# emmanuel-ferdman/pinot

Measured on AMD Instinct MI355X. Metric: rows scanned/s (G) + p50 query latency, SSB flattened SF100/SF1000, 1-8 GPU, higher is better.
Workload: dtype u32 dict ids / int64 sums; 1 GPU; SSB SF100 flattened lineorder per GPU, 100 segments x 6000000 rows, queries Q1.1+Q1.2+Q1.3; layout=sorted by LO_ORDERDATE (SURVEY.md §8d C2), rows_per_gpu=600000000, parallelism=one GPU (no collective)

## Files before the change

### pinot_amd/csrc/device.h

```cpp
#pragma once
#include <stdint.h>

#if defined(__HIPCC__)
#define PHIP_HD __host__ __device__
#else
#define PHIP_HD
#endif

namespace phip {

constexpr int kMaxQueryColumns = 16;
constexpr int kMaxAggs = 8;
constexpr int kRecKeys = 4;
constexpr int kRecFields = kRecKeys + 2 * kMaxAggs;
enum { REC_BITS = 0, REC_U16 = 1, REC_U32 = 2 };
struct RecSrc {
  const void *p;
  int32_t kind, bits, off, pad;
};
struct RecSrcs {
  RecSrc f[kRecFields];
};
constexpr int kMaxPrograms = 8;
constexpr int kDenseMin = 640;
constexpr int kDoneSlot = 63;
constexpr int kMaxFilterStack = 6;
constexpr int kMaxGroupBy = 8;
constexpr int kWave = 64;
constexpr int kTileGroups = 32;
constexpr int kTileDocs = kTileGroups * 64;
constexpr int kMaxStage = 8;
constexpr int kStagePad = 16;
constexpr int kMaxHllRegs = 1 << 12;

constexpr int kFilterBlock = 256;
constexpr int kFilterWaves = kFilterBlock / kWave;
constexpr int kMaxRing = 8;
constexpr int kFilterStaticLds = 448;
constexpr int kFusedRingTile = 512;
#ifndef PHIP_FUSED_RING_DEFER
#define PHIP_FUSED_RING_DEFER 512
#endif
constexpr int kFusedRingDefer = PHIP_FUSED_RING_DEFER;
constexpr int kAggBlock = 512;
constexpr int kAggWaves = kAggBlock / kWave;
#ifndef PHIP_KBATCH
#define PHIP_KBATCH 4
#endif
constexpr int kRingAgg = PHIP_KBATCH <= 4 ? 1024 : 2048;
constexpr int kRingGroup = 128;
constexpr int kRingGroupBatch = PHIP_KBATCH <= 4 ? 512 : 1024;
constexpr int kFusedRingGB = 256;
constexpr int kFusedBatchGB = 2;
constexpr int ring_entries(int mode, bool batched = false) {
  return mode == 0 ? kRingAgg : (batched ? kRingGroupBatch : kRingGroup);
}
constexpr int kMaxAggStage = 4;
constexpr int kAggStageBudget = 4096;
constexpr int kAggLdsDict = 1024;

enum AccKind : int32_t {
  ACC_COUNT = 0,
  ACC_SUM_I64 = 1,
  ACC_SUM_F64 = 2,
  ACC_MIN_F64 = 3,
  ACC_MAX_F64 = 4,
  ACC_HLL = 5,
  ACC_DISTINCT = 6,
};

enum DevOp : int32_t { DOP_LEAF = 0, DOP_AND = 1, DOP_OR = 2, DOP_NOT = 3 };
enum SkipKind : int32_t { SKIP_NONE = 0, SKIP_IF_NONE = 1, SKIP_IF_ALL = 2 };

enum GroupMode : int32_t {
  GB_NONE = 0,
  GB_LDS = 1,
  GB_GLOBAL = 2,
  GB_HASH = 3,
  GB_XCD = 4,
};
constexpr int kXcdCopies = 8;
constexpr int kFusedGroupBy = -1;
constexpr int kFusedGroupByXcd = -2;
constexpr int kFusedGroupByLds = -3;
constexpr uint64_t kHashEmpty = ~0ull;

struct DevCol {
  const uint32_t *words;
  const void *dict;
  const void *raw;
  const int32_t *remap;
  const uint32_t *hll;
  int32_t bits;
  int32_t card;
  int32_t type;
  int32_t has_dict;
  int32_t lds_off;
  int32_t hll_rows;
  const uint64_t *str_off;
  const uint32_t *planes;
  int64_t gb_base;
  const uint32_t *hll_doc;
  const uint16_t *hll_doc16;
  const uint64_t *gb_nulls;
  int64_t gb_null_id;
  const int32_t *gb_ids;
  const uint32_t *vpack;
  int64_t vbase;
  int32_t vbits;
  int32_t vpad;
};
constexpr int kBitSliceMaxBits = 12;

constexpr int kExprMaxOps = 32;
constexpr int kExprMaxStack = 8;
constexpr int kExprMaxCols = 8;
constexpr int kMaxDerivedPerSegment = 16;
enum ExprOp : int32_t { EXOP_COLUMN = 0, EXOP_CONST = 1, EXOP_ADD = 2, EXOP_SUB = 3, EXOP_MUL = 4, EXOP_DIV = 5 };
struct DevExprOp {
  int32_t op;
  int32_t col;
  int64_t lval;
  double dval;
};
struct DevExpr {
  int32_t num_ops;
  int32_t num_docs;
  DevExprOp ops[kExprMaxOps];
  DevCol cols[kExprMaxCols];
};

struct MvScanTask {
  const uint32_t *words;
  const uint32_t *offsets;
  const uint32_t *set;
  uint64_t *out;
  int32_t tile_words;
  int32_t num_docs;
  int32_t num_tiles;
  int32_t tile_begin;
  int32_t bits;
  int32_t lo, hi;
  int32_t invert;
  int32_t set_words;
  int32_t pad;
};
struct MvReduceTask {
  const uint32_t *words;
  const uint32_t *offsets;
  const void *dict;
  void *out;
  int32_t num_docs;
  int32_t bits;
  int32_t type;
  int32_t kind;
  int32_t integral;
  int32_t pad;
};

constexpr int kMaxTupleCols = 8;
constexpr int kMaxTupleWords = 4;
struct TupleCol {
  const uint32_t *words;
  const int32_t *remap;
  const int32_t *ids;
  const void *raw;
  const uint64_t *nulls;
  int64_t base;
  int64_t null_id;
  uint64_t stride;
  int32_t bits;
  int32_t type;
  int32_t word;
  int32_t pad;
};
struct TupleCols {
  TupleCol cols[kMaxTupleCols];
  int32_t k;
  int32_t w;
};

struct StageSrc {
  const uint8_t *base;
  int32_t bytes;
  int32_t lds_off;
};

#ifndef PHIP_MAX_CONJ
#define PHIP_MAX_CONJ 6
#endif
constexpr int kMaxConj = PHIP_MAX_CONJ;
constexpr int kConjSparseMax = 6;
constexpr double kConjSparseSel = 1.0 / 16;
struct ConjLeaf {
  int32_t lds_off;
  int32_t bits;
  int32_t kind;
  uint32_t lo;
  uint32_t span;
  int32_t pad;
  uint64_t set_mask;
};

struct DevSeg {
  int32_t num_docs;
  int32_t work_begin;
  int32_t tile0;
  int32_t num_work;
  int32_t node_begin;
  int32_t node_end;
  int32_t num_stage;
  int32_t seg_index;
  int32_t num_dma;
  int32_t conj;
  int32_t conj_p;
  int32_t conj_sparse;
  int32_t conj_path;
  int32_t conj_range;
  int32_t conj_lo;
  int32_t conj_hi;
  int32_t contig;
  int32_t program;
  int32_t fused_defer;
  int32_t conj_bs;
  ConjLeaf conj_leaf[kMaxConj];
  StageSrc stage[kMaxStage];
  DevCol cols[kMaxQueryColumns];
  const uint32_t *rec;
  int32_t rec_words;
  int32_t rec_nf;
  uint8_t rec_off[kRecFields];
  uint8_t rec_bits[kRecFields];
};

struct DevNode {
  int32_t op;
  int32_t leaf_kind;
  int32_t column;
  int32_t lo, hi;
  int32_t exclusive;
  int32_t count;
  int32_t skip_to;
  int32_t skip_kind;
  int32_t lds_off;
  int32_t bits;
  int32_t small_set;
  int32_t aux_stride;
  uint64_t set_mask;
  int32_t bs_nruns;
  uint32_t bs_runs[4];
  const void *aux;
};

constexpr int kFinShards = 16;
constexpr size_t kFinCounterBytes = 64 * (1 + kFinShards);
struct DevFinal {
  const uint64_t *pa;
  const int32_t *ka;
  const uint64_t *pf;
  const int32_t *kf;
  uint64_t *segm;
  uint32_t *hll;
  uint64_t *out;
  uint32_t *counter;
  int32_t nba, na, nbf, nseg, hll_words, pad;
};

struct DevFilter {
  const DevSeg *segs;
// ... 203 lines not shown
```

### pinot_amd/csrc/filter_kernel.h

```cpp
#pragma once
#include <hip/hip_ext.h>

#include "agg_kernel.h"
#include "host_final.h"

namespace phip {

struct Tile {
  int32_t doc0;
  int32_t valid_docs;
  const PHIP_LDS uint8_t *stage;
};

#define PHIP_GROUP_LOOP(PASS_EXPR)                                             \
  const int lane = lane_id();                                                  \
  const int32_t p = lane * B;                                                  \
  const int32_t q = (p - 1) >> 5;                                              \
  const uint32_t s = (uint32_t)(32 * (q + 1) - p);                             \
  const PHIP_LDS uint32_t *wl = w + q;                                         \
  const int32_t gstride = 2 * B;                                               \
  uint32_t r = 0;                                                              \
  _Pragma("unroll 8") for (int g = 0; g < kTileGroups; g++) {                  \
    const uint32_t win = __builtin_amdgcn_alignbit(wl[0], wl[1], s);           \
    wl += gstride;                                                             \
// ... 1071 lines not shown
static_assert(kFusedRingDefer - 64 * lean_batch(1) >= 32 * defer_piece_lanes(kFusedRingDefer - 64 * lean_batch(1)),
              "a piece fits the ring beside a lean batch");

template <int NA, int U = kFusedBatch>
__device__ __forceinline__ void fused_defer(cquery_t &aq, cseg_t &seg, const Tile &t, uint32_t mask,
                                            PHIP_LDS uint32_t *ring, int &head, int &tail, const SmallDict (&sda)[NA],
                                            const SmallDict (&sdb)[NA], uint64_t (&acc)[NA]) {
  constexpr int kDeferPieceLanes = defer_piece_lanes(kFusedRingDefer - 64 * U);
  if (ballot(mask != 0) == 0) return;
  const TileRank r = rank_tile(mask);
  const int head0 = head;
  const int npiece = head - tail + r.total <= kFusedRingDefer ? 1 : 64 / kDeferPieceLanes;
  const int lanes = 64 / npiece;
  for (int p = 0; p < npiece; p++) {
    const int e = __builtin_amdgcn_readlane((int)r.incl, lanes * p + lanes - 1);
    write_ranked<uint32_t, kFusedRingDefer>(r, lanes * p, lanes * (p + 1), -head0, t.doc0, ring);
    head = head0 + e;
    while (head - tail >= 64 * U) {
      fused_flush<NA, U>(aq, seg, ring, tail, 64 * U, sda, sdb, acc);
      tail += 64 * U;
    }
  }
}

constexpr int kGbFlush = 64 * kFusedBatchGB;
static_assert(kFusedRingGB >= 2 * kGbFlush, "a piece of <= kGbFlush docs lands on < kGbFlush pending");

template <int MODE>
__device__ __forceinline__ void fused_flush_gb(cquery_t &aq, cseg_t &seg, const PHIP_LDS uint32_t *ring, int tail, int n,
                                               lds_u64 *tbl, lds_u32 *hll_packed) {
  group_ring_batch<MODE, kFusedBatchGB, kFusedRingGB>(aq, seg, (const lds_u32 *)ring, tail, n, tbl, hll_packed);
}

template <int MODE>
__device__ __forceinline__ void fused_defer_gb(cquery_t &aq, cseg_t &seg, const Tile &t, uint32_t mask,
                                               PHIP_LDS uint32_t *ring, int &head, int &tail, lds_u64 *tbl,
                                               lds_u32 *hll_packed) {
  if (ballot(mask != 0) == 0) return;
  const TileRank r = rank_tile(mask);
  const int head0 = head;
  const int npiece = head - tail + r.total <= kFusedRingGB ? 1 : 16;
  const int lanes = 64 / npiece;
  for (int p = 0; p < npiece; p++) {
    const int e = __builtin_amdgcn_readlane((int)r.incl, lanes * p + lanes - 1);
    write_ranked<uint32_t, kFusedRingGB>(r, lanes * p, lanes * (p + 1), -head0, t.doc0, ring);
    head = head0 + e;
    while (head - tail >= kGbFlush) {
      fused_flush_gb<MODE>(aq, seg, ring, tail, kGbFlush, tbl, hll_packed);
      tail += kGbFlush;
    }
  }
}

#define PHIP_VMW(k) \
  case k: asm volatile("s_waitcnt vmcnt(" #k ")" ::: "memory"); break;
__device__ __forceinline__ void wait_vmcnt_lb(int n) {
  switch (__builtin_amdgcn_readfirstlane(n)) {
    PHIP_VMW(0) PHIP_VMW(1) PHIP_VMW(2) PHIP_VMW(3) PHIP_VMW(4) PHIP_VMW(5) PHIP_VMW(6) PHIP_VMW(7)
    PHIP_VMW(8) PHIP_VMW(9) PHIP_VMW(10) PHIP_VMW(11) PHIP_VMW(12) PHIP_VMW(13) PHIP_VMW(14)
    default: asm volatile("s_waitcnt vmcnt(15)" ::: "memory"); break;
  }
}
#undef PHIP_VMW

template <int kS>
struct StageCursor {
  const uint8_t *ptr[kS];
  int32_t bytes[kS];
  int32_t lds[kS];
  int32_t n;
};

template <int kS>
__device__ __forceinline__ void cursor_load(StageCursor<kS> &c, cseg_t &seg, int32_t tile_in_seg) {
  c.n = seg.num_stage;
#pragma unroll
  for (int i = 0; i < kS; i++) {
    c.ptr[i] = nullptr;
    c.bytes[i] = 0;
    c.lds[i] = 0;
    if (i < c.n) {
      c.bytes[i] = seg.stage[i].bytes;
      c.lds[i] = seg.stage[i].lds_off;
      c.ptr[i] = seg.stage[i].base + (int64_t)tile_in_seg * c.bytes[i];
    }
  }
}

template <int kS>
__device__ __forceinline__ void cursor_issue(StageCursor<kS> &c, uint32_t lbase, int step) {
  const int lane16 = lane_id() * 16;
#pragma unroll
  for (int i = 0; i < kS; i++) {
    if (i < c.n) {
      const uint8_t *g = c.ptr[i] + lane16;
      const uint32_t l = lbase + (uint32_t)c.lds[i];
      const int32_t nb = c.bytes[i];
      for (int off = 0; off < nb; off += 1024) {
        if (off + lane16 < nb) dma16(g + off, l + (uint32_t)off);
      }
      c.ptr[i] += (int64_t)nb * step;
    }
  }
}

template <int NA>
__device__ __forceinline__ void record_store(const DevFilter &q, const uint64_t *part, const uint64_t *apart,
                                             const uint32_t *segrow) {
  const int i = (int)threadIdx.x;
  if (i >= (q.rec_stride >> 3)) return;
  int na = 0;
  if constexpr (NA > 0) na = ((cquery_t *)q.agg)->num_aggs;
  uint64_t v = 0;
  if (i < 2) {
    for (int w = 0; w < kFilterWaves; w++) v += part[w * 2 + i];
  } else if (i < 2 + 2 * na) {
    if constexpr (NA > 0) {
      const int a = (i - 2) >> 1, kind = ((cquery_t *)q.agg)->aggs[a].acc;
      v = apart[a];
      for (int w = 1; w < kFilterWaves; w++) v = acc_combine(kind, v, apart[w * NA + a]);
      v = (i & 1) ? (v >> 48) : v;
    }
  } else {
    const int e = q.rec_first[blockIdx.x] + (i - 2 - 2 * na);
    for (int w = 0; w < kFilterWaves; w++) v += segrow[w * kRecSegSlots + e % kRecSegSlots];
  }
  __hip_atomic_store(q.rec + (((size_t)blockIdx.x * (uint32_t)q.rec_stride) >> 3) + i, rec_word(q.rec_tag, v),
                     __ATOMIC_RELAXED, __HIP_MEMORY_SCOPE_SYSTEM);
}

#ifndef PHIP_FUSED_WAVES
#define PHIP_FUSED_WAVES 5
#endif
template <bool kConjOnly, int NA, bool kBsDefer = false>
__global__ __launch_bounds__(kFilterBlock, kConjOnly ? (NA != 0 ? PHIP_FUSED_WAVES : 6) : 4) void filter_kernel(DevFilter q) {
  static_assert(!kBsDefer || (kConjOnly && NA > 0), "the lean shape is a fused aggregation");
  constexpr int kSConj = kBsDefer ? kMaxConj : (NA > 0 ? kMaxConj + kMaxAggStage : kMaxConj);
  constexpr int kS = kConjOnly ? (kSConj < kMaxStage ? kSConj : kMaxStage) : kMaxStage;
  extern __shared__ __attribute__((aligned(16))) unsigned char smem[];
  const int lane = lane_id();
  const int wave = uniform(threadIdx.x >> 6);
  int begin, end, step;
  if (q.xcd_walk == 1) {
    const int x = blockIdx.x & 7, gx = gridDim.x >> 3;
    begin = (int)((int64_t)q.total_work * x / 8) + (int)(blockIdx.x >> 3) * kFilterWaves + wave;
    end = (int)((int64_t)q.total_work * (x + 1) / 8);
    step = gx * kFilterWaves;
  } else {
    const TileRange r = wave_tile_range(q.xcd_walk, q.total_work, (int)gridDim.x, (int)blockIdx.x, wave, kFilterWaves);
    begin = r.begin;
    end = r.end;
    step = 1;
  }
  const int nbuf = q.nbuf;
  const int stride = q.stage_stride;
  PHIP_LDS uint8_t *ring = (PHIP_LDS uint8_t *)(smem + (size_t)wave * nbuf * stride);
  PHIP_LDS uint8_t *docring_b = (PHIP_LDS uint8_t *)(smem + (size_t)kFilterWaves * nbuf * stride) +
                                (NA != 0 ? (size_t)wave * q.fring_bytes : 0);
  PHIP_LDS uint16_t *docring = (PHIP_LDS uint16_t *)docring_b;
  PHIP_LDS uint32_t *deferring = (PHIP_LDS uint32_t *)docring_b;
  int dhead = 0, dtail = 0;
  const uint32_t ring_lds = __builtin_amdgcn_readfirstlane((uint32_t)(uintptr_t)ring);

  cseg_t *segs = (cseg_t *)q.segs;
  cnode_t *nodes = (cnode_t *)q.nodes;
  uint32_t lane_matched = 0;
  uint64_t scanned = 0;
  uint64_t matched_total = 0;
  const int nd = q.min_dma;
  const int st = kBsDefer ? 0 : (q.mask_out != nullptr ? 1 : 0);
  constexpr int NAX = NA > 0 ? NA : 1;
  constexpr int kB = kBsDefer ? lean_batch(NA) : kFusedBatch;
  constexpr int kGbMode = NA == kFusedGroupByXcd ? GB_XCD : (NA == kFusedGroupByLds ? GB_LDS : GB_GLOBAL);
  lds_u64 *gtbl = nullptr;
  lds_u32 *ghll = nullptr;
  if constexpr (NA == kFusedGroupByLds) {
    cquery_t &aq = *(cquery_t *)q.agg;
    gtbl = (lds_u64 *)(smem + (size_t)kFilterWaves * (nbuf * stride + q.fring_bytes));
    ghll = (lds_u32 *)((PHIP_LDS uint8_t *)gtbl + (size_t)aq.tbl_words * 8);
    const int G = (int)aq.num_groups;
    for (int i = threadIdx.x; i < aq.tbl_words; i += kFilterBlock) {
      const int row = i / G;
      gtbl[i] = (row > 0 && aq.aggs[row - 1].acc == ACC_MIN_F64) ? ~0ull : 0ull;
    }
    for (int i = threadIdx.x; i < aq.hll_words; i += kFilterBlock) ghll[i] = 0;
    __syncthreads();
  }
  __shared__ uint32_t segrow[kFilterWaves][NA >= 0 ? kRecSegSlots : 1];
  if constexpr (NA >= 0) {
    segrow[wave][min(lane, kRecSegSlots - 1)] = 0;
  }
  uint64_t acc[NAX];
  SmallDict sda[NAX], sdb[NAX];
  if constexpr (NA > 0) {
    cquery_t &aq = *(cquery_t *)q.agg;
#pragma unroll
    for (int a = 0; a < NA; a++) {
      acc[a] = a < aq.num_aggs ? acc_init(aq.aggs[a].acc) : 0;
      sda[a] = sdb[a] = SmallDict{0u, 0u, false};
    }
  }

  int pf = begin, pfc = 0, psn = 0, pend = -1, pslot = 0;
  StageCursor<kS> cur;
  cur.n = 0;
#define PHIP_PREFETCH()                                                                         \
  do {                                                                                          \
    if (pf >= pend) {                                                                           \
      while (psn + 1 < q.num_segs && segs[psn].work_begin + segs[psn].num_work <= pf) psn++;    \
      cseg_t &ps = segs[psn];                                                                   \
      pend = ps.work_begin + ps.num_work;                                                       \
      cursor_load<kS>(cur, ps, ps.tile0 + (pf - ps.work_begin));                                \
    }                                                                                           \
    cursor_issue<kS>(cur, ring_lds + (uint32_t)(pslot * stride), step);                         \
    pf += step;                                                                                 \
    pfc++;                                                                                      \
// ... 186 lines not shown
```

### pinot_amd/csrc/runtime.cpp

```cpp
#include <hip/hip_runtime.h>

#include <algorithm>
#include <atomic>
#include <chrono>
#include <condition_variable>
#include <cmath>
#include <cstdarg>
#include <cstdio>
#include <cstring>
#include <functional>
#include <map>
#include <memory>
#include <mutex>
#include <string>
#include <unordered_map>
#include <vector>

#include "../../include/pinot_hip.h"
#include "device.h"
#include "host_final.h"
#include "launch.h"
#include "node.h"

using namespace phip;

static thread_local std::string g_err;

static int32_t fail(int32_t code, const char *fmt, ...) {
  char buf[1024];
  va_list ap;
  va_start(ap, fmt);
  vsnprintf(buf, sizeof(buf), fmt, ap);
  va_end(ap);
  g_err = buf;
  return code;
}

#define HIP_TRY(expr)                                                                         \
  do {                                                                                        \
    hipError_t _e = (expr);                                                                   \
    if (_e != hipSuccess) return fail(PHIP_ERR_HIP, "%s failed: %s", #expr, hipGetErrorString(_e)); \
  } while (0)

static inline int64_t ceil_div(int64_t a, int64_t b) { return (a + b - 1) / b; }
static inline int64_t round_up(int64_t a, int64_t b) { return ceil_div(a, b) * b; }
static inline uint32_t be32(const uint8_t *p) {
  return ((uint32_t)p[0] << 24) | ((uint32_t)p[1] << 16) | ((uint32_t)p[2] << 8) | p[3];
}
static inline uint64_t be64(const uint8_t *p) { return ((uint64_t)be32(p) << 32) | be32(p + 4); }
static inline uint32_t le32(const uint8_t *p) {
  return (uint32_t)p[0] | ((uint32_t)p[1] << 8) | ((uint32_t)p[2] << 16) | ((uint32_t)p[3] << 24);
}
static inline uint16_t le16(const uint8_t *p) { return (uint16_t)(p[0] | (p[1] << 8)); }

static int num_bits_per_value(int32_t max_value) {
  if (max_value <= 1) return 1;
  int b = 0;
  while (max_value > 0) {
    b++;
    max_value >>= 1;
  }
  return b;
}

static int type_width(int32_t t) {
  switch (t) {
    case PHIP_TYPE_INT:
    case PHIP_TYPE_FLOAT: return 4;
    case PHIP_TYPE_LONG:
    case PHIP_TYPE_DOUBLE: return 8;
    default: return 0;
  }
}

static int32_t murmur_hash_long(int64_t data) {
  const uint32_t m = 0x5bd1e995u;
  uint32_t h = 0;
  uint32_t k = (uint32_t)data * m;
  k ^= k >> 24;
  h ^= k * m;
  k = (uint32_t)((uint64_t)data >> 32) * m;
  k ^= k >> 24;
  h *= m;
  h ^= k * m;
  h ^= h >> 13;
  h *= m;
  h ^= h >> 15;
  return (int32_t)h;
}
static int32_t murmur_hash_bytes(const uint8_t *d, int32_t len, int32_t seed) {
  const uint32_t m = 0x5bd1e995u;
  uint32_t h = (uint32_t)seed ^ (uint32_t)len;
  int32_t n4 = len >> 2;
  for (int32_t i = 0; i < n4; i++) {
    uint32_t k = le32(d + 4 * i);
    k *= m;
    k ^= k >> 24;
    k *= m;
    h *= m;
    h ^= k;
  }
// ... 3636 lines not shown
  int64_t mv_total_tiles = 0, mv_entries = 0;
  for (size_t i = 0; i < inv_leaves.size(); i++) {
    const InvLeaf &L = inv_leaves[i];
    const ColumnStore &cs = segs[L.seg]->cols[L.col];
    uint64_t *words = (uint64_t *)inv_words + inv_word_off[i];
    const int32_t tile_words = 32 * entry_leaves[L.entry];
    nodes[L.node].aux = words;
    nodes[L.node].aux_stride = tile_words;
    node_inv_stride[L.node] = tile_words;
    node_inv_slot[L.node] = L.slot;
    node_inv_leaves[L.node] = entry_leaves[L.entry];
    if (L.mv) {
      if (!entry_has_work[L.entry]) continue;
      MvScanTask t;
      memset(&t, 0, sizeof(t));
      t.words = cs.words;
      t.offsets = cs.mv_off;
      t.out = words;
      t.tile_words = tile_words;
      t.num_docs = segs[L.seg]->num_docs;
      t.num_tiles = (int32_t)(inv_word_nw[i] / 32);
      t.tile_begin = mv_total_tiles;
      t.bits = cs.bits;
      t.lo = L.mv_lo;
      t.hi = L.mv_hi;
      t.invert = L.mv_invert;
      t.set_words = L.mv_set_words;
      mv_total_tiles += t.num_tiles;
      if (mv_total_tiles > INT32_MAX / 2) return fail(PHIP_ERR_UNSUPPORTED, "too many multi-value scan tiles in one query");
      if (L.mv_stats) mv_entries += cs.total_values;
      mv_tasks.push_back(t);
      mv_set_offs.push_back(L.mv_set_words > 0 ? L.mv_set_off : SIZE_MAX);
      continue;
    }
    const size_t first = tasks.size();
    for (int k = 0; k < L.src->count; k++) {
      int32_t id = L.src->ids[k];
      if (id < 0 || id >= cs.card) return fail(PHIP_ERR_INVALID, "inverted dict id %d out of range", id);
      for (int64_t ci = cs.inv_begin[id]; ci < cs.inv_begin[id + 1]; ci++) {
        const Container &ct = cs.inv_conts[ci];
        RoaringTask t;
        t.payload = cs.inv_blob + ct.off;
        t.out_words = words;
        t.key = ct.key;
        t.kind = ct.kind;
        t.card = ct.card;
        t.pad = 0;
        tasks.push_back(t);
      }
    }
    std::stable_sort(tasks.begin() + first, tasks.end(),
                     [](const RoaringTask &a, const RoaringTask &b) { return a.key < b.key; });
    if (tasks.size() > (size_t)INT32_MAX) return fail(PHIP_ERR_UNSUPPORTED, "too many inverted-index containers");
    const int32_t nkeys = (int32_t)(inv_word_nw[i] / 1024);
    size_t t = first;
    for (int32_t key = 0; key < nkeys; key++) {
      size_t e = t;
      while (e < tasks.size() && tasks[e].key == key) e++;
      RoaringGroup g;
      g.out_words = words;
      g.task_begin = (int32_t)t;
      g.task_end = (int32_t)e;
      g.key = key;
      g.tile_words = tile_words;
      rgroups.push_back(g);
      t = e;
    }
    if (t != tasks.size()) return fail(PHIP_ERR_INVALID, "inverted-index container key beyond the segment's docs");
  }
  const size_t tasks_off = tasks.empty() ? 0 : blob.add(tasks.data(), tasks.size() * sizeof(RoaringTask));
  const size_t rgroups_off = rgroups.empty() ? 0 : blob.add(rgroups.data(), rgroups.size() * sizeof(RoaringGroup));
  const size_t mv_tasks_off = mv_tasks.empty() ? 0 : blob.reserve(mv_tasks.size() * sizeof(MvScanTask));

  bool has_filter = false;
  for (const DevSeg &ds : dsegs) has_filter |= ds.node_end > ds.node_begin;
  bool need_agg = group_by || nprog > 1;
  for (int a = 0; a < naggs; a++) need_agg |= dq.aggs[a].acc != ACC_COUNT;
  const int ndist = (int)P.dist_agg.size();
  bool need_mask = has_filter && (need_agg || want_bitmap || nsel > 0 || ndist > 0);
  const int64_t kSlotBudget = 19 * 1024;
  int32_t stage_stride = 0;
  std::vector<double> seg_est(dsegs.size(), 1.0);
  std::vector<int32_t> seg_off(dsegs.size(), 0);
  for (DevSeg &ds : dsegs) {
    int32_t off = 0;
    ds.num_stage = 0;
    ds.num_dma = 0;
    auto add_region = [&](const uint8_t *rbase, int32_t bytes) -> int32_t {
      if (ds.num_stage >= kMaxStage || off + bytes + 2 * kStagePad > kSlotBudget) return -1;
      const int32_t lds_off = off + kStagePad;
      ds.stage[ds.num_stage++] = {rbase, bytes, lds_off};
      ds.num_dma += (int32_t)ceil_div(bytes, 1024);
      off += bytes + 2 * kStagePad;
      return lds_off;
    };
    int32_t inv_region = -2;
    bool bs = getenv("PHIP_NO_BITSLICE") == nullptr && ds.node_end > ds.node_begin;
    for (int i = ds.node_begin; i < ds.node_end && bs; i++) {
      const DevNode &dn = nodes[i];
      if (dn.op == DOP_AND || (dn.op == DOP_LEAF && dn.leaf_kind == PHIP_LEAF_MATCH_ALL)) continue;
      if (dn.op == DOP_LEAF && dn.leaf_kind == PHIP_LEAF_DOC_RANGES && dn.count == 1) continue;
      bs = dn.op == DOP_LEAF && (dn.leaf_kind == PHIP_LEAF_DICT_RANGE || dn.leaf_kind == PHIP_LEAF_DICT_SET) &&
           ds.cols[dn.column].planes != nullptr &&
           (dn.leaf_kind == PHIP_LEAF_DICT_RANGE || bs_small_set(dn, ds.cols[dn.column]) || bs_runs_set(dn));
    }
    if (bs) {
      std::vector<int> cols_seen;
      int64_t need = 0;
      for (int i = ds.node_begin; i < ds.node_end; i++) {
        const DevNode &dn = nodes[i];
        if (dn.op != DOP_LEAF || (dn.leaf_kind != PHIP_LEAF_DICT_RANGE && dn.leaf_kind != PHIP_LEAF_DICT_SET)) continue;
        if (std::find(cols_seen.begin(), cols_seen.end(), dn.column) != cols_seen.end()) continue;
        cols_seen.push_back(dn.column);
        need += 256ll * ds.cols[dn.column].bits + 2 * kStagePad;
      }
      bs = (int)cols_seen.size() <= kMaxStage && need <= kSlotBudget;
    }
    std::vector<std::pair<int, int32_t>> bs_regions;
    for (int i = ds.node_begin; i < ds.node_end; i++) {
      DevNode &dn = nodes[i];
      if (dn.op != DOP_LEAF) continue;
      if (bs && (dn.leaf_kind == PHIP_LEAF_DICT_RANGE || dn.leaf_kind == PHIP_LEAF_DICT_SET)) {
        const DevCol &dc = ds.cols[dn.column];
        int32_t r = -2;
        for (const auto &p : bs_regions) r = p.first == dn.column ? p.second : r;
        if (r == -2) {
          r = add_region((const uint8_t *)dc.planes, 256 * dc.bits);
          bs_regions.push_back({dn.column, r});
        }
        dn.lds_off = r;
        continue;
      }
      if (dn.leaf_kind == PHIP_LEAF_DICT_RANGE || dn.leaf_kind == PHIP_LEAF_DICT_SET) {
        DevCol &dc = ds.cols[dn.column];
        if (dc.lds_off < 0) dc.lds_off = add_region((const uint8_t *)dc.words, 256 * dc.bits);
        dn.lds_off = dc.lds_off;
      } else if (dn.leaf_kind == PHIP_LEAF_INVERTED && dn.aux != nullptr && node_inv_leaves[i] == 0) {
        dn.lds_off = add_region((const uint8_t *)dn.aux, 256);
      } else if (dn.leaf_kind == PHIP_LEAF_INVERTED && dn.aux != nullptr) {
        if (inv_region == -2) {
          const uint64_t *entry_base = (const uint64_t *)dn.aux - 32 * node_inv_slot[i];
          inv_region = add_region((const uint8_t *)entry_base, 256 * node_inv_leaves[i]);
        }
        dn.lds_off = inv_region < 0 ? -1 : inv_region + 256 * node_inv_slot[i];
      }
    }
    stage_stride = std::max(stage_stride, off);
    ds.conj = 0;
    ds.conj_path = 0;
    ds.conj_range = 0;
    ds.conj_lo = 0;
    ds.conj_hi = ds.num_docs - 1;
    std::vector<std::pair<double, ConjLeaf>> conj;
    bool ok = true;
    double est = 1.0;
    for (int i = ds.node_begin; i < ds.node_end && ok; i++) {
      const DevNode &dn = nodes[i];
      if (dn.op == DOP_AND) continue;
      if (dn.op == DOP_LEAF && dn.leaf_kind == PHIP_LEAF_MATCH_ALL) continue;
      if (dn.op == DOP_LEAF && dn.leaf_kind == PHIP_LEAF_DOC_RANGES && dn.count == 1) {
        ds.conj_range = 1;
        ds.conj_lo = std::max(ds.conj_lo, dn.lo);
        ds.conj_hi = std::min(ds.conj_hi, dn.hi);
        est *= double(std::max(0, dn.hi - dn.lo + 1)) / std::max(1, ds.num_docs);
        continue;
      }
      if (dn.op != DOP_LEAF || dn.lds_off < 0 ||
          !(dn.leaf_kind == PHIP_LEAF_DICT_RANGE || (dn.leaf_kind == PHIP_LEAF_DICT_SET && dn.small_set) ||
            (bs && bs_runs_set(dn)))) {
        ok = false;
        break;
      }
      const int card = std::max(1, ds.cols[dn.column].card);
      ConjLeaf L;
      memset(&L, 0, sizeof(L));
      L.lds_off = dn.lds_off;
      L.bits = dn.bits;
      double sel;
      if (bs && dn.leaf_kind == PHIP_LEAF_DICT_SET && bs_runs_set(dn)) {
        L.kind = 4;
        L.set_mask = (uint64_t)dn.bs_runs[0] | ((uint64_t)dn.bs_runs[1] << 32);
        L.lo = dn.bs_runs[2];
        L.span = dn.bs_runs[3];
        L.pad = dn.bs_nruns;
        int64_t n = 0;
        for (int r = 0; r < dn.bs_nruns; r++) n += (int64_t)(dn.bs_runs[r] >> 16) - (dn.bs_runs[r] & 0xffff) + 1;
        sel = double(n) / card;
      } else if (bs && dn.leaf_kind == PHIP_LEAF_DICT_SET) {
        L.kind = 3;
        L.set_mask = dn.set_mask & (card >= 64 ? ~0ull : ((1ull << card) - 1));
        sel = double(__builtin_popcountll(L.set_mask)) / card;
      } else if (bs) {
        L.kind = 2;
        L.lo = (uint32_t)dn.lo;
        L.span = (uint32_t)(dn.hi - 1);
        L.pad = (dn.lo > 0 ? 1 : 0) | (dn.hi < card ? 2 : 0);
        sel = double(dn.hi - dn.lo) / card;
      } else if (dn.leaf_kind == PHIP_LEAF_DICT_RANGE) {
        L.kind = 0;
        L.lo = (uint32_t)dn.lo << (32 - dn.bits);
        L.span = (uint32_t)(dn.hi - dn.lo) << (32 - dn.bits);
        sel = double(dn.hi - dn.lo) / card;
      } else {
        L.kind = 1;
        L.set_mask = dn.set_mask;
        const uint64_t in_dict = card >= 64 ? ~0ull : ((1ull << card) - 1);
        sel = double(__builtin_popcountll(dn.set_mask & in_dict)) / card;
      }
      est *= sel;
      conj.push_back({sel, L});
    }
    if (ds.conj_range && ds.conj_lo > ds.conj_hi) ok = false;
    if (ok && (int)conj.size() <= kMaxConj) {
      ds.conj_path = 1;
      seg_est[&ds - dsegs.data()] = est;
      std::stable_sort(conj.begin(), conj.end(),
                       [](const std::pair<double, ConjLeaf> &a, const std::pair<double, ConjLeaf> &b) { return a.first < b.first; });
      ds.conj = (int32_t)conj.size();
      ds.conj_bs = bs ? 1 : 0;
      ds.conj_sparse = bs ? 0 : 1;
      for (size_t i = 1; i < conj.size(); i++) ds.conj_sparse &= conj[i].second.kind == 0 ? 1 : 0;
      if (conj.empty() || conj[0].first > kConjSparseSel) ds.conj_sparse = 0;
      if (getenv("PHIP_NO_SPARSE")) ds.conj_sparse = 0;
      if (ds.conj_sparse) {
        const char *sm = getenv("PHIP_SPARSE_MAX");
        ds.conj_sparse = sm ? std::max(1, std::min(32, atoi(sm))) : kConjSparseMax;
      }
      ds.conj_p = 8;
      for (size_t i = 0; i < conj.size(); i++) {
        ds.conj_leaf[i] = conj[i].second;
        while (ds.conj_p > 1 && ds.conj_p * conj[i].second.bits > 32) ds.conj_p >>= 1;
      }
      if (const char *e = getenv("PHIP_CONJ_P")) ds.conj_p = std::min(ds.conj_p, std::max(1, atoi(e)));
    }
    ds.contig = 0;
    if (!ds.conj_path && ds.node_end > ds.node_begin) {
      bool c = true;
      for (int i = ds.node_begin; i < ds.node_end && c; i++) {
        const DevNode &dn = nodes[i];
        if (dn.op != DOP_LEAF) continue;
        switch (dn.leaf_kind) {
          case PHIP_LEAF_MATCH_ALL:
          case PHIP_LEAF_MATCH_NONE:
          case PHIP_LEAF_DOC_RANGES: break;
          case PHIP_LEAF_INVERTED: c = dn.lds_off >= 0; break;
          case PHIP_LEAF_DICT_RANGE: c = dn.lds_off >= 0 && dn.bits >= 1 && dn.bits <= 31; break;
          case PHIP_LEAF_DICT_SET:
            c = dn.lds_off >= 0 && dn.bits >= 1 && dn.bits <= 31 && (dn.small_set || (dn.count > 0 && dn.count <= 64));
            break;
          default: c = false;
        }
      }
      const char *ce = getenv("PHIP_CONTIG");
      ds.contig = c && !(ce && ce[0] == '0') ? 1 : 0;
    }
    seg_off[&ds - dsegs.data()] = off;
  }
  if (rec_want) {
    bool made = false;
    for (size_t i = 0; i < dsegs.size(); i++) {
      const int s = dsegs[i].seg_index % nseg;
      int32_t rc = build_records(*segs[s], q, dq, dsegs[i], colidx[s], rec_min_fields, seg_est[i], st, &made);
      if (rc) return rc;
    }
    if (made) HIP_TRY(hipStreamSynchronize(st));
    int64_t rec_docs = 0, all_docs = 0;
    for (const DevSeg &d : dsegs) {
      all_docs += d.num_docs;
      rec_docs += d.rec != nullptr ? d.num_docs : 0;
    }
    if (rec_min_fields > 1 && 2 * rec_docs < all_docs)
      for (DevSeg &d : dsegs) d.rec = nullptr;
  }
  bool conj_all = true;
  for (const DevSeg &ds : dsegs) conj_all &= ds.conj_path != 0;
  bool any_filter_prog = false;
  for (const DevSeg &ds : dsegs) any_filter_prog |= ds.node_end > ds.node_begin;
  int fused_naggs = 0;
  bool any_defer = false;
  std::vector<bool> ids_streamed((size_t)nseg * ncols, false);
  {
    const char *fe = getenv("PHIP_FUSE");
    const int64_t kFuseMaxTiles = 8192;
    double est_docs = 0.0;
    for (size_t i = 0; i < dsegs.size(); i++) est_docs += seg_est[i] * dsegs[i].num_docs;
    const double per_tile = est_docs / (double)std::max<int64_t>(1, total_work);
    double fuse_per_tile = 0.0;
    if (const char *fp = getenv("PHIP_FUSE_PER_TILE")) fuse_per_tile = atof(fp);
    const bool big = total_work > kFuseMaxTiles;
    const double kFuseDenseSplit = 1024.0;
    const bool dense_small = !big && per_tile >= kFuseDenseSplit;
    const char *fl = getenv("PHIP_FUSE_LARGE");
    bool bs_all = true;
    for (const DevSeg &ds : dsegs) bs_all &= ds.conj == 0 || ds.conj_bs != 0;
    const bool fuse_large = (fl ? atoi(fl) != 0 : true) && bs_all;
    bool fuse = conj_all && any_filter_prog && !group_by && nprog == 1 && nhll == 0 && naggs > 0 && naggs <= 4 && !want_bitmap &&
                ndist == 0 &&
                (fe ? atoi(fe) != 0 : (!dense_small && (!big || fuse_large || (fuse_per_tile > 0 && per_tile <= fuse_per_tile))));
    bool any_value = false;
    for (int a = 0; a < naggs; a++) any_value |= dq.aggs[a].acc != ACC_COUNT;
    if (fuse && any_value) {
      fused_naggs = naggs;
      const char *sv = getenv("PHIP_STREAM_VALUES");
      const char *sp = getenv("PHIP_STREAM_PACKED");
      const double kStreamValueMin = 0.5;
      for (size_t i = 0; i < dsegs.size(); i++) {
        DevSeg &ds = dsegs[i];
        int32_t off = seg_off[i];
        const int32_t nstage0 = ds.num_stage;
        for (int a = 0; a < naggs; a++) {
          const DevAgg &ag = dq.aggs[a];
          if (ag.acc == ACC_COUNT) continue;
          for (int c : {ag.col_a, ag.expr != PHIP_EXPR_COLUMN ? ag.col_b : -1}) {
            if (c < 0) continue;
            DevCol &dc = ds.cols[c];
            if (dc.lds_off >= 0) continue;
            const int sidx = ds.seg_index % nseg;
            const ColumnStore &cs = segs[sidx]->cols[colidx[sidx][c]];
            const bool via_vals = !dc.has_dict && !no_dict(cs);
            if (!dc.has_dict && !via_vals) continue;
            const bool via_packed = via_vals && dc.vpack != nullptr && !(sp && atoi(sp) == 0);
            const int32_t bits = via_packed ? dc.vbits : via_vals ? cs.bits : dc.bits;
            const bool dense = seg_est[i] * (1024.0 / std::max(1, bits)) >= kStreamValueMin;
            if (!(sv ? atoi(sv) != 0 : (dense && !big))) continue;
            const int32_t bytes = 256 * bits;
            if (ds.num_stage >= std::min(kMaxStage, kMaxConj + kMaxAggStage) || off + bytes + 2 * kStagePad > kSlotBudget)
              continue;
            if (via_vals && !via_packed) {
              dc.has_dict = 1;
              dc.raw = cs.raw;
              dc.vpack = nullptr;
              dc.vbits = 0;
              ids_streamed[(size_t)sidx * ncols + c] = true;
            }
            dc.lds_off = off + kStagePad;
            ds.stage[ds.num_stage++] = {(const uint8_t *)(via_packed ? dc.vpack : dc.words), bytes, dc.lds_off};
            ds.num_dma += (int32_t)ceil_div(bytes, 1024);
            off += bytes + 2 * kStagePad;
          }
        }
        stage_stride = std::max(stage_stride, off);
        ds.fused_defer = ds.num_stage == nstage0 ? 1 : 0;
        if (const char *fd = getenv("PHIP_FUSED_DEFER")) ds.fused_defer = ds.fused_defer && atoi(fd) != 0;
        any_defer |= ds.fused_defer != 0;
      }
    }
  }
  bool fused_gb = false, gb_xcd = false, gb_lds = false;
  int64_t gb_lds_bytes = 0;
  if (group_by && dq.mode != GB_HASH && conj_all && any_filter_prog && nprog == 1 && !want_bitmap && nsel == 0 &&
      ndist == 0) {
    const char *fg = getenv("PHIP_FUSED_GB");
    const int fgm = fg ? atoi(fg) : 1;
    const int64_t m = nhll ? ((int64_t)1 << log2m) : 0;
    const int64_t table_bytes = (int64_t)(1 + naggs) * dq.num_groups * 8 + (int64_t)nhll * dq.num_groups * m;
    const char *force = getenv("PHIP_GB_MODE");
    const bool lds_sized = table_bytes <= 128 * 1024 && !(force && !strcmp(force, "global"));
    double est_docs = 0.0;
    for (size_t i = 0; i < dsegs.size(); i++) est_docs += seg_est[i] * dsegs[i].num_docs;
    const double per_key = est_docs / (double)std::max<int64_t>(1, dq.num_groups);
    const double kFuseGbMaxPerKey = 40.0;
    const char *fx = getenv("PHIP_FUSED_GB_XCD_MAX");
    const int64_t xcd_max = fx ? atoll(fx) : (int64_t)16 << 20;
    bool sorted_key = false;
    for (int k = 0; k < q->num_group_by; k++)
      for (int s2 = 0; s2 < nseg; s2++)
        sorted_key |= !segs[s2]->cols[colidx[s2][q->group_by_columns[k]]].sorted_pairs.empty();
    fused_gb = fgm == 2 || fgm == 3 || (fgm == 1 && (!lds_sized || (per_key <= kFuseGbMaxPerKey && !sorted_key)));
    gb_xcd = fused_gb && fgm != 2 && table_bytes <= xcd_max && (fgm == 3 || per_key >= 1.0) &&
             dev->num_xcc <= kXcdCopies;
    if (fgm == 4 && lds_sized) {
      const int64_t lb = round_up((int64_t)(1 + naggs) * dq.num_groups * 8 + (int64_t)nhll * dq.num_groups * m, 16);
      const int64_t ss = round_up(std::max(stage_stride, 16), 16);
      if ((160 * 1024 - 256 - (int64_t)kFilterWaves * 4 * kFusedRingGB - lb) / ((int64_t)kFilterWaves * ss) >= 2) {
        fused_gb = gb_lds = true;
        gb_xcd = false;
        gb_lds_bytes = lb;
      }
    }
    if (fused_gb) {
      any_defer = true;
      for (DevSeg &ds : dsegs) ds.fused_defer = 1;
    }
  }
  stage_stride = (int32_t)round_up(std::max(stage_stride, 16), 16);
  for (const DevSeg &ds : dsegs) {
    int64_t per_tile = 0;
    std::vector<int> seen;
    for (int i = ds.node_begin; i < ds.node_end; i++) {
      const DevNode &dn = nodes[i];
      if (dn.op != DOP_LEAF) continue;
      if (dn.leaf_kind == PHIP_LEAF_DICT_RANGE || dn.leaf_kind == PHIP_LEAF_DICT_SET) {
        if (std::find(seen.begin(), seen.end(), dn.column) == seen.end()) {
          seen.push_back(dn.column);
          per_tile += 256ll * ds.cols[dn.column].bits;
        }
      } else if (dn.leaf_kind == PHIP_LEAF_INVERTED) {
        per_tile += 256;
      } else if (dn.leaf_kind == PHIP_LEAF_RAW_RANGE || dn.leaf_kind == PHIP_LEAF_RAW_SET) {
        per_tile += (int64_t)kTileDocs * type_width(ds.cols[dn.column].type);
      } else if (dn.leaf_kind == PHIP_LEAF_RAW_STRING_RANGE || dn.leaf_kind == PHIP_LEAF_RAW_STRING_SET) {
        const int s = ds.seg_index % nseg;
        const ColumnStore &cs = segs[s]->cols[colidx[s][dn.column]];
        per_tile += (int64_t)kTileDocs * 8 + (int64_t)(kTileDocs * cs.str_total / std::max<int64_t>(segs[s]->num_docs, 1));
      }
    }
    P.filter_bytes += per_tile * ds.num_work;
  }
  for (int c = 0; c < ncols; c++) {
    if (!projected[c]) continue;
    Plan::ProjCol pc;
    pc.progs = proj_progs[c];
    for (int s = 0; s < nseg; s++) {
      const ColumnStore &cs = segs[s]->cols[colidx[s][c]];
      const bool raw = (as_raw(s, c) && !ids_streamed[(size_t)s * ncols + c]) || hll_doc_used[(size_t)s * ncols + c];
      const bool packed = raw && !no_dict(cs) && !hll_doc_used[(size_t)s * ncols + c] && packed_vals(cs);
      pc.bits.push_back(packed ? cs.vbits : raw ? 0 : cs.bits);
      pc.card.push_back(raw ? 0 : cs.card);
      pc.width.push_back(hll_doc16_used[(size_t)s * ncols + c] ? 2 : (cs.type == PHIP_TYPE_STRING ? 4 : type_width(cs.type)));
    }
    P.proj.push_back(pc);
  }
  for (int s = 0; s < nseg; s++) P.seg_docs.push_back(segs[s]->num_docs);
  const bool conj_only = conj_all;
  if (fused_naggs > 0 || fused_gb) need_mask = false;
  const bool fused_any = fused_naggs > 0 || fused_gb;
  bool fused_lean = fused_naggs > 0 && !fused_gb && conj_only;
  for (const DevSeg &ds : dsegs)
    fused_lean = fused_lean && (ds.conj == 0 || ds.conj_bs != 0) && ds.fused_defer == 1 && ds.num_stage <= kMaxConj;
  if (const char *le = getenv("PHIP_FUSED_LEAN")) fused_lean = fused_lean && atoi(le) != 0;
  int nbuf = 0, fbpc = 0;
  int grid_cus = dev->num_cus;
  if (const char *gc = getenv("PHIP_GRID_CUS")) {
    if (atoi(gc) >= 1) {
      grid_cus = atoi(gc);
      P.sel_max_blocks = (int)std::min<int64_t>(4096, (int64_t)grid_cus * 8);
    }
  }
  const int32_t fring_bytes = fused_gb ? 4 * kFusedRingGB : (any_defer ? 4 * kFusedRingDefer : 2 * kFusedRingTile);
  {
    const char *env = getenv("PHIP_FILTER_BPC");
    int want = env ? std::max(1, std::min(8, atoi(env))) : (conj_only ? 6 : 4);
    const int64_t kMinTilesPerWave = 12;
    const int64_t waves_at = (int64_t)grid_cus * want * kFilterWaves;
    if (!env && total_work >= 4 * waves_at && !fused_any)
      while (want > 2 && total_work < kMinTilesPerWave * (int64_t)grid_cus * want * kFilterWaves) want--;
    const int64_t fring = (fused_any ? (int64_t)kFilterWaves * fring_bytes : 0) + gb_lds_bytes;
    const int64_t static_lds = fused_gb ? 256 : kFilterStaticLds;
    for (int bpc = want; bpc >= 1 && nbuf < 2; bpc--) {
      const int64_t nb = std::min<int64_t>(kMaxRing, ((160 * 1024) / bpc - static_lds - fring) / ((int64_t)kFilterWaves * stage_stride));
      if (nb >= 2) {
        nbuf = (int)nb;
        fbpc = bpc;
      }
    }
    if (nbuf < 2) return fail(PHIP_ERR_UNSUPPORTED, "filter needs %d bytes of LDS per ring slot", stage_stride);
    const char *fs = getenv("PHIP_FUSED_SMALL");
    if (!env && fused_any && !(fs && atoi(fs) == 0) &&
        total_work <= (int64_t)dev->num_cus * kFilterWaves * 8 && fbpc > 1) {
      const int64_t nb = std::min<int64_t>(kMaxRing, ((160 * 1024) - static_lds - fring) / ((int64_t)kFilterWaves * stage_stride));
      if (nb >= 2) {
        nbuf = (int)nb;
        fbpc = 1;
      }
    }
  }
  const size_t filter_lds = (size_t)kFilterWaves * nbuf * stage_stride + (fused_any ? (size_t)kFilterWaves * fring_bytes : 0) +
                            (size_t)gb_lds_bytes;
  const char *walk_env = getenv("PHIP_FILTER_WALK");
  int xcd_walk = fused_any ? 2 : 0;
  if (walk_env) xcd_walk = !strcmp(walk_env, "xcd") ? 1 : (!strcmp(walk_env, "xcdc") ? 2 : 0);
  int64_t min_tiles_per_wave = 1;
  if (const char *mt = getenv("PHIP_FILTER_MIN_TILES")) min_tiles_per_wave = std::max(1, atoi(mt));
  int filter_blocks = (int)std::max<int64_t>(1, std::min<int64_t>((int64_t)grid_cus * fbpc,
                                                                  ceil_div(total_work, kFilterWaves * min_tiles_per_wave)));
  if (xcd_walk) filter_blocks = (int)round_up(std::max(filter_blocks, 8), 8);

  dq.log2m = log2m;
  if (dq.mode != GB_HASH) dq.mode = group_by ? GB_GLOBAL : GB_NONE;
  if (group_by) dq.dense_batch = 0;
  const int m_regs = nhll ? (1 << log2m) : 0;
  size_t agg_lds = (size_t)kAggWaves * ring_entries(dq.mode) * 4 + (size_t)kAggWaves * dq.stage_bytes;
  int agg_bpc = 4;
  void *first_doc = nullptr;
  if (group_by && dq.mode == GB_HASH && nseg == 1 && gb_key_space >= q->num_groups_limit && q->num_groups_limit > 0) {
    int32_t rc0 = P.alloc((size_t)dq.num_groups * 4, &first_doc);
    if (rc0) return rc0;
    dq.seg_keys = 1;
    dq.seg_key_mult = 1;
    dq.first_doc = (uint32_t *)first_doc;
  }
  if (group_by && dq.mode == GB_HASH) {
    if ((int64_t)nhll * dq.num_groups * m_regs * 4 > ((int64_t)16 << 30))
      return fail(PHIP_ERR_UNSUPPORTED, "DISTINCTCOUNTHLL registers of %lld hash slots exceed the memory budget",
                  (long long)dq.num_groups);
  } else if (group_by) {
    const int64_t tbl_words = (int64_t)(1 + naggs) * dq.num_groups;
    const int64_t hll_words = (int64_t)nhll * dq.num_groups * m_regs / 4;
    const int64_t table_bytes = tbl_words * 8 + hll_words * 4;
    const char *force = getenv("PHIP_GB_MODE");
    bool use_lds = table_bytes <= 128 * 1024 && (!fused_gb || gb_lds);
    if (force && !strcmp(force, "global")) use_lds = false;
    if (force && !strcmp(force, "lds") && !fused_gb && (int64_t)agg_lds + round_up(table_bytes, 16) <= 159 * 1024)
      use_lds = true;
    const char *gbb = getenv("PHIP_GB_BATCH");
    const int64_t tb = round_up(table_bytes, 16);
    const int64_t ring_extra = (int64_t)kAggWaves * (kRingGroupBatch - kRingGroup) * 4;
    auto bpc_of = [&](int64_t lds) { return std::max<int64_t>(1, std::min<int64_t>(4, (160 * 1024 - 1024) / lds)); };
    bool batched = use_lds && bpc_of((int64_t)agg_lds + ring_extra + tb) >= bpc_of((int64_t)agg_lds + tb);
    if (gbb) batched = atoi(gbb) != 0;
    if (use_lds && (int64_t)agg_lds + ring_extra + tb > 159 * 1024) batched = false;
    dq.dense_batch = batched ? 1 : 0;
    agg_lds = (size_t)kAggWaves * ring_entries(dq.mode == GB_HASH ? GB_HASH : GB_LDS, batched) * 4 +
              (size_t)kAggWaves * dq.stage_bytes;
    if (use_lds) {
      dq.mode = GB_LDS;
      dq.tbl_words = (int32_t)tbl_words;
      dq.hll_words = (int32_t)hll_words;
      const char *gw = getenv("PHIP_GB_WAVES");
      auto walk_of = [&](bool b) {
        Plan::GbWalk w;
        w.batched = b;
        w.lds = (size_t)kAggWaves * ring_entries(GB_LDS, b) * 4 + (size_t)kAggWaves * dq.stage_bytes +
                (size_t)round_up(table_bytes, 16);
        int bpc = std::max(1, std::min(4, (int)((160 * 1024 - 1024) / w.lds)));
// ... 2427 lines not shown
```

Before: 10960 G rows/s.

## Stage only the needed high bit planes for bit-sliced range leaves

For bit-sliced dictionary range filters, the host now finds how many low-order bit planes can never change the range result, from the trailing zeros of lo and trailing ones of hi-1. It stages only the remaining high planes into LDS, keeps the full per-tile advance through a packed copy/advance field, and shifts the leaf bounds and bit width to match. This cuts DMA traffic and LDS footprint per tile for the sorted-date SSB predicates. It also caps the requested blocks per CU for fused conjunctive aggregations at the fused-waves launch bound. The risk is a correctness dependence on the pruning math and on the packed 16-bit byte counts.

Result: no change. 11060 G rows/s (median of 3 runs) (+0.9%).

```diff
diff --git a/pinot_amd/csrc/bs_prune.h b/pinot_amd/csrc/bs_prune.h
--- /dev/null
+++ b/pinot_amd/csrc/bs_prune.h
@@ -0,0 +1,15 @@
+#pragma once
+#include <cstdint>
+
+inline int bs_prune_planes(int B, uint32_t lo, uint32_t hi, int sides) {
+  int t = B;
+  if (sides & 1) {
+    const int z = lo ? __builtin_ctz(lo) : B;
+    t = z < t ? z : t;
+  }
+  if (sides & 2) {
+    const int o = ~hi ? __builtin_ctz(~hi) : B;
+    t = o < t ? o : t;
+  }
+  return t;
+}
diff --git a/pinot_amd/csrc/device.h b/pinot_amd/csrc/device.h
--- a/pinot_amd/csrc/device.h
+++ b/pinot_amd/csrc/device.h
@@ -37,6 +37,10 @@
 constexpr int kFilterWaves = kFilterBlock / kWave;
 constexpr int kMaxRing = 8;
 constexpr int kFilterStaticLds = 448;
+#ifndef PHIP_FUSED_WAVES
+#define PHIP_FUSED_WAVES 5
+#endif
+constexpr int kFusedWaves = PHIP_FUSED_WAVES;
 constexpr int kFusedRingTile = 512;
 #ifndef PHIP_FUSED_RING_DEFER
 #define PHIP_FUSED_RING_DEFER 512
@@ -185,6 +189,9 @@
   int32_t bytes;
   int32_t lds_off;
 };
+constexpr int32_t stage_pack(int32_t copy, int32_t advance) { return copy | (advance << 16); }
+constexpr int32_t stage_copy(int32_t packed) { return packed & 0xffff; }
+constexpr int32_t stage_advance(int32_t packed) { return (int32_t)((uint32_t)packed >> 16); }
 
 #ifndef PHIP_MAX_CONJ
 #define PHIP_MAX_CONJ 6
diff --git a/pinot_amd/csrc/filter_kernel.h b/pinot_amd/csrc/filter_kernel.h
--- a/pinot_amd/csrc/filter_kernel.h
+++ b/pinot_amd/csrc/filter_kernel.h
@@ -1177,7 +1177,7 @@
     if (i < c.n) {
       c.bytes[i] = seg.stage[i].bytes;
       c.lds[i] = seg.stage[i].lds_off;
-      c.ptr[i] = seg.stage[i].base + (int64_t)tile_in_seg * c.bytes[i];
+      c.ptr[i] = seg.stage[i].base + (int64_t)tile_in_seg * stage_advance(c.bytes[i]);
     }
   }
 }
@@ -1190,11 +1190,11 @@
     if (i < c.n) {
       const uint8_t *g = c.ptr[i] + lane16;
       const uint32_t l = lbase + (uint32_t)c.lds[i];
-      const int32_t nb = c.bytes[i];
+      const int32_t nb = stage_copy(c.bytes[i]);
       for (int off = 0; off < nb; off += 1024) {
         if (off + lane16 < nb) dma16(g + off, l + (uint32_t)off);
       }
-      c.ptr[i] += (int64_t)nb * step;
+      c.ptr[i] += (int64_t)stage_advance(c.bytes[i]) * step;
     }
   }
 }
@@ -1224,9 +1224,6 @@
                      __ATOMIC_RELAXED, __HIP_MEMORY_SCOPE_SYSTEM);
 }
 
-#ifndef PHIP_FUSED_WAVES
-#define PHIP_FUSED_WAVES 5
-#endif
 template <bool kConjOnly, int NA, bool kBsDefer = false>
 __global__ __launch_bounds__(kFilterBlock, kConjOnly ? (NA != 0 ? PHIP_FUSED_WAVES : 6) : 4) void filter_kernel(DevFilter q) {
   static_assert(!kBsDefer || (kConjOnly && NA > 0), "the lean shape is a fused aggregation");
diff --git a/pinot_amd/csrc/runtime.cpp b/pinot_amd/csrc/runtime.cpp
--- a/pinot_amd/csrc/runtime.cpp
+++ b/pinot_amd/csrc/runtime.cpp
@@ -17,6 +17,7 @@
 #include <vector>
 
 #include "../../include/pinot_hip.h"
+#include "bs_prune.h"
 #include "device.h"
 #include "host_final.h"
 #include "launch.h"
@@ -3819,14 +3820,15 @@
   int32_t stage_stride = 0;
   std::vector<double> seg_est(dsegs.size(), 1.0);
   std::vector<int32_t> seg_off(dsegs.size(), 0);
+  std::vector<std::vector<std::pair<int, int32_t>>> seg_bs_bytes(dsegs.size());
   for (DevSeg &ds : dsegs) {
     int32_t off = 0;
     ds.num_stage = 0;
     ds.num_dma = 0;
-    auto add_region = [&](const uint8_t *rbase, int32_t bytes) -> int32_t {
+    auto add_region = [&](const uint8_t *rbase, int32_t bytes, int32_t advance = 0) -> int32_t {
       if (ds.num_stage >= kMaxStage || off + bytes + 2 * kStagePad > kSlotBudget) return -1;
       const int32_t lds_off = off + kStagePad;
-      ds.stage[ds.num_stage++] = {rbase, bytes, lds_off};
+      ds.stage[ds.num_stage++] = {rbase, stage_pack(bytes, advance ? advance : bytes), lds_off};
       ds.num_dma += (int32_t)ceil_div(bytes, 1024);
       off += bytes + 2 * kStagePad;
       return lds_off;
@@ -3853,17 +3855,49 @@
       }
       bs = (int)cols_seen.size() <= kMaxStage && need <= kSlotBudget;
     }
-    std::vector<std::pair<int, int32_t>> bs_regions;
+    bool prune = bs;
+    if (const char *pe = getenv("PHIP_BS_PRUNE")) prune = prune && atoi(pe) != 0;
+    if (prune) {
+      int nleaf = 0;
+      for (int i = ds.node_begin; i < ds.node_end; i++)
+        nleaf += nodes[i].op == DOP_LEAF &&
+                 (nodes[i].leaf_kind == PHIP_LEAF_DICT_RANGE || nodes[i].leaf_kind == PHIP_LEAF_DICT_SET);
+      prune = nleaf <= kMaxConj;
+    }
+    struct BsRegion {
+      int column;
+      int32_t lds_off;
+      int32_t t;
+    };
+    std::vector<BsRegion> bs_regions;
     for (int i = ds.node_begin; i < ds.node_end; i++) {
       DevNode &dn = nodes[i];
       if (dn.op != DOP_LEAF) continue;
       if (bs && (dn.leaf_kind == PHIP_LEAF_DICT_RANGE || dn.leaf_kind == PHIP_LEAF_DICT_SET)) {
         const DevCol &dc = ds.cols[dn.column];
         int32_t r = -2;
-        for (const auto &p : bs_regions) r = p.first == dn.column ? p.second : r;
+        for (const BsRegion &p : bs_regions) r = p.column == dn.column ? p.lds_off : r;
         if (r == -2) {
-          r = add_region((const uint8_t *)dc.planes, 256 * dc.bits);
-          bs_regions.push_back({dn.column, r});
+          int32_t t = prune ? dc.bits - 1 : 0;
+          for (int j = ds.node_begin; j < ds.node_end && t > 0; j++) {
+            const DevNode &o = nodes[j];
+            if (o.op != DOP_LEAF || o.column != dn.column) continue;
+            if (o.leaf_kind == PHIP_LEAF_DICT_SET) t = 0;
+            if (o.leaf_kind != PHIP_LEAF_DICT_RANGE) continue;
+            if (o.hi <= o.lo) {
+              t = 0;
+              continue;
+            }
+            const int sides = (o.lo > 0 ? 1 : 0) | (o.hi < std::max(1, dc.card) ? 2 : 0);
+            const int lt = bs_prune_planes(dc.bits, (uint32_t)o.lo, (uint32_t)(o.hi - 1), sides);
+            if (sides != 0 && lt >= dc.bits)
+              return fail(PHIP_ERR_INVALID, "bit-sliced leaf [%d, %d) of a %d-bit column tests a side and no plane", o.lo,
+                          o.hi, dc.bits);
+            t = std::min(t, lt);
+          }
+          r = add_region((const uint8_t *)dc.planes, 256 * (dc.bits - t), 256 * dc.bits);
+          bs_regions.push_back({dn.column, r, t});
+          seg_bs_bytes[&ds - dsegs.data()].push_back({dn.column, 256 * (dc.bits - t)});
         }
         dn.lds_off = r;
         continue;
@@ -3928,9 +3962,12 @@
         L.set_mask = dn.set_mask & (card >= 64 ? ~0ull : ((1ull << card) - 1));
         sel = double(__builtin_popcountll(L.set_mask)) / card;
       } else if (bs) {
+        int32_t t = 0;
+        for (const BsRegion &p : bs_regions) t = p.column == dn.column ? p.t : t;
         L.kind = 2;
-        L.lo = (uint32_t)dn.lo;
-        L.span = (uint32_t)(dn.hi - 1);
+        L.bits = dn.bits - t;
+        L.lo = (uint32_t)dn.lo >> t;
+        L.span = (uint32_t)(dn.hi - 1) >> t;
         L.pad = (dn.lo > 0 ? 1 : 0) | (dn.hi < card ? 2 : 0);
         sel = double(dn.hi - dn.lo) / card;
       } else if (dn.leaf_kind == PHIP_LEAF_DICT_RANGE) {
@@ -4071,7 +4108,8 @@
               ids_streamed[(size_t)sidx * ncols + c] = true;
             }
             dc.lds_off = off + kStagePad;
-            ds.stage[ds.num_stage++] = {(const uint8_t *)(via_packed ? dc.vpack : dc.words), bytes, dc.lds_off};
+            ds.stage[ds.num_stage++] = {(const uint8_t *)(via_packed ? dc.vpack : dc.words), stage_pack(bytes, bytes),
+                                        dc.lds_off};
             ds.num_dma += (int32_t)ceil_div(bytes, 1024);
             off += bytes + 2 * kStagePad;
           }
@@ -4130,7 +4168,9 @@
       if (dn.leaf_kind == PHIP_LEAF_DICT_RANGE || dn.leaf_kind == PHIP_LEAF_DICT_SET) {
         if (std::find(seen.begin(), seen.end(), dn.column) == seen.end()) {
           seen.push_back(dn.column);
-          per_tile += 256ll * ds.cols[dn.column].bits;
+          int64_t staged = 256ll * ds.cols[dn.column].bits;
+          for (const auto &p : seg_bs_bytes[&ds - dsegs.data()]) staged = p.first == dn.column ? p.second : staged;
+          per_tile += staged;
         }
       } else if (dn.leaf_kind == PHIP_LEAF_INVERTED) {
         per_tile += 256;
@@ -4178,6 +4218,7 @@
   {
     const char *env = getenv("PHIP_FILTER_BPC");
     int want = env ? std::max(1, std::min(8, atoi(env))) : (conj_only ? 6 : 4);
+    if (!env && fused_any && conj_only) want = std::min(want, kFusedWaves);
     const int64_t kMinTilesPerWave = 12;
     const int64_t waves_at = (int64_t)grid_cus * want * kFilterWaves;
     if (!env && total_work >= 4 * waves_at && !fused_any)
```
